# ska-sa/katsdpsigproc

Measured on AMD Instinct MI355X. Metric: visibility samples/s (baselines x channels) through full RFI flagger, higher is better.
Workload: dtype f32 amplitude / f64 deviations

## Files before the change

### katsdpsigproc_amd/csrc/fused_common.h

```cpp
#pragma once
#include <stdlib.h>

#include "bitplane.h"
#include "median_merge.h"
#include "median_window.h"

#ifndef FUSED_MAD_BITS
#define FUSED_MAD_BITS 1
#endif
#ifndef FUSED_STRIP
#define FUSED_STRIP 4
#endif
#define FUSED_THREADS (64 * FUSED_STRIP)
#define FUSED_MAD_NORMAL 1.4826

#ifdef KSP_DIAG_REALTIME
#define FUSED_DIAG_CLOCK() __builtin_amdgcn_s_memrealtime()
#else
#define FUSED_DIAG_CLOCK() __builtin_amdgcn_s_memtime()
#endif
#ifdef KSP_DIAG
#define FUSED_DIAG_STOP(p) ((p).debug_stop)
#define FUSED_DIAG_TRACE(p) ((p).trace)
#else
#define FUSED_DIAG_STOP(p) 0
#define FUSED_DIAG_TRACE(p) ((unsigned long long *)nullptr)
#endif

struct FusedParams {
    const void *vis;
    const uint8_t *in_flags;
    uint8_t *flags;
    float *deviations;
    float *noise;
    int channels, baselines;
    int vis_stride, in_flags_stride, flags_stride, dev_stride;
    int is_amplitude, flags_mode, threshold_kind, n_windows, flag_value;
    int n_strips;
    int n_static, n_dyn, dyn_blocks;
    unsigned *work;
    int first_round;
#ifdef KSP_DIAG
    int debug_stop;
    unsigned long long *trace;
#endif
    double n_sigma;
    double scales[KSP_MAX_WINDOWS];
};

template <int R>
struct FusedLayout {
    static constexpr int RUN = R + 4;
    static constexpr int ROW = 64 * RUN + 8;
    static constexpr int LDS_FLOATS = FUSED_STRIP * ROW;
    static constexpr int LIST_DOUBLES = 256;
    static constexpr size_t LDS_BYTES =
        sizeof(float) * LDS_FLOATS + sizeof(double) * LIST_DOUBLES * FUSED_STRIP;
    __device__ static __forceinline__ int index(int c) { return (c / R) * RUN + (c % R); }
};

#ifndef FUSED_XCD_GROUP
#define FUSED_XCD_GROUP 8
#endif
__device__ __forceinline__ int strip_of(int id, int n_strips)
{
    constexpr int G = FUSED_XCD_GROUP;
    const int full = (n_strips / (8 * G)) * (8 * G);
    if (id >= full) return id;
    const int xcd = id & 7, i = id >> 3;
    return ((i / G) * 8 + xcd) * G + (i % G);
}

__device__ __forceinline__ float amp_with_flags(const FusedParams &p, float re, float im,
                                                int row, int bl)
{
    float a = ksp_abs_c64(re, im);
    if (p.flags_mode == KSP_FLAGS_CHANNEL) {
        if (p.in_flags[row]) a = __builtin_nanf("");
    } else if (p.flags_mode == KSP_FLAGS_FULL) {
        if (p.in_flags[(size_t)row * p.in_flags_stride + bl]) a = __builtin_nanf("");
    }
    return a;
}

template <int R>
__device__ __forceinline__ void load_strip(const FusedParams &p, float *lds, int b0, int tid)
{
    using LY = FusedLayout<R>;
    constexpr int LB = 4;
    constexpr int LPR = FUSED_STRIP / 2;
    constexpr int RSTEP = FUSED_THREADS / LPR;
    const int C = p.channels;
    const int q = tid % LPR;
    const int r0 = tid / LPR;
    const int bl = b0 + 2 * q;
    const bool ok0 = bl < p.baselines, ok1 = bl + 1 < p.baselines;
    const bool plain = !p.is_amplitude && ok1;
    auto request = [&](float4 (&raw)[LB], unsigned (&fl)[LB], int rbase) {
#pragma unroll
        for (int u = 0; u < LB; u++) {
            const int row = rbase + u * RSTEP;
            raw[u] = make_float4(0.f, 0.f, 0.f, 0.f);
            fl[u] = 0;
            if (plain && row < C) {
                raw[u] = *(const float4 *)((const float2 *)p.vis + (size_t)row * p.vis_stride + bl);
                if (p.flags_mode == KSP_FLAGS_CHANNEL) {
                    fl[u] = p.in_flags[row];
                } else if (p.flags_mode == KSP_FLAGS_FULL) {
                    fl[u] = *(const unsigned short *)(p.in_flags + (size_t)row * p.in_flags_stride + bl);
                }
            }
        }
    };
    auto finish = [&](const float4 (&raw)[LB], const unsigned (&fl)[LB], int rbase) {
#pragma unroll
        for (int u = 0; u < LB; u++) {
            const int row = rbase + u * RSTEP;
            if (row >= C) break;
            float a0 = __builtin_nanf(""), a1 = __builtin_nanf("");
            unsigned fl8;
            if (plain) {
                a0 = ksp_abs_c64(raw[u].x, raw[u].y);
                a1 = ksp_abs_c64(raw[u].z, raw[u].w);
                if (p.flags_mode == KSP_FLAGS_CHANNEL) fl8 = fl[u] ? 0x101u : 0u; else fl8 = fl[u];
                if (fl8 & 0xffu) a0 = __builtin_nanf("");
                if (fl8 >> 8) a1 = __builtin_nanf("");
            } else if (p.is_amplitude) {
                const float *src = (const float *)p.vis + (size_t)row * p.vis_stride + bl;
                if (ok0) a0 = src[0];
                if (ok1) a1 = src[1];
                if (p.flags_mode == KSP_FLAGS_CHANNEL) {
                    if (p.in_flags[row]) a0 = a1 = __builtin_nanf("");
                } else if (p.flags_mode == KSP_FLAGS_FULL) {
                    const uint8_t *f = p.in_flags + (size_t)row * p.in_flags_stride + bl;
                    if (ok0 && f[0]) a0 = __builtin_nanf("");
                    if (ok1 && f[1]) a1 = __builtin_nanf("");
                }
            } else if (ok0) {
                const float2 v = ((const float2 *)p.vis)[(size_t)row * p.vis_stride + bl];
                a0 = amp_with_flags(p, v.x, v.y, row, bl);
            }
            const int idx = LY::index(row);
            lds[(2 * q) * LY::ROW + idx] = a0;
            lds[(2 * q + 1) * LY::ROW + idx] = a1;
        }
    };
    constexpr int BATCH = RSTEP * LB;
    float4 bufa[LB], bufb[LB];
    unsigned fla[LB], flb[LB];
    request(bufa, fla, r0);
    for (int rbase = r0; rbase < C; rbase += 2 * BATCH) {
        if (rbase + BATCH < C) request(bufb, flb, rbase + BATCH);
        finish(bufa, fla, rbase);
        if (rbase + BATCH < C) {
            if (rbase + 2 * BATCH < C) request(bufa, fla, rbase + 2 * BATCH);
            finish(bufb, flb, rbase + BATCH);
        }
    }
    for (int row = C + r0; row < 64 * R; row += RSTEP) {
        const int idx = LY::index(row);
        lds[(2 * q) * LY::ROW + idx] = __builtin_nanf("");
        lds[(2 * q + 1) * LY::ROW + idx] = __builtin_nanf("");
    }
}

#ifndef FUSED_LOAD_LB
#define FUSED_LOAD_LB 4
#endif
#ifndef FUSED_LOAD_NB
#define FUSED_LOAD_NB 3
#endif
template <int R, int MODE>
__device__ __forceinline__ bool load_strip_fast(const FusedParams &p, float *lds, int b0, int tid)
{
    using LY = FusedLayout<R>;
    constexpr int LB = FUSED_LOAD_LB;
    constexpr int LPR = FUSED_STRIP / 2;
    constexpr int RSTEP = FUSED_THREADS / LPR;
    constexpr int BATCH = RSTEP * LB;
    const int C = p.channels;
    const int q = tid % LPR;
    const int r0 = tid / LPR;
    const int bl = b0 + 2 * q;
    const float2 *vis = (const float2 *)p.vis + bl;
    const size_t stride = (size_t)p.vis_stride;
    unsigned umax = 0, flag_or = 0;
    auto request = [&](float4 (&raw)[LB], unsigned (&fl)[LB], int rbase) {
#pragma unroll
        for (int u = 0; u < LB; u++) {
            const int row = min(rbase + r0 + u * RSTEP, C - 1);
            raw[u] = *(const float4 *)(vis + (size_t)row * stride);
            fl[u] = 0;
            if (MODE == KSP_FLAGS_CHANNEL)
                fl[u] = p.in_flags[row];
            else if (MODE == KSP_FLAGS_FULL)
                fl[u] = *(const unsigned short *)(p.in_flags + (size_t)row * p.in_flags_stride + bl);
        }
    };
    auto finish = [&](const float4 (&raw)[LB], const unsigned (&fl)[LB], int rbase) {
        float amp[LB][2];
        if (FUSED_DIAG_STOP(p) == 11) {
#pragma unroll
            for (int u = 0; u < LB; u++) {
                amp[u][0] = raw[u].x;
                amp[u][1] = raw[u].z;
            }
        } else {
            ksp_abs_c64_batch<LB, MODE == KSP_FLAGS_NONE>(raw, amp, umax);
        }
#pragma unroll
        for (int u = 0; u < LB; u++) {
            const int row = rbase + r0 + u * RSTEP;
            float a0 = amp[u][0], a1 = amp[u][1];
            if (MODE == KSP_FLAGS_CHANNEL) {
                if (fl[u]) a0 = a1 = __builtin_nanf("");
            } else if (MODE == KSP_FLAGS_FULL) {
                if (fl[u] & 0xffu) a0 = __builtin_nanf("");
                if (fl[u] >> 8) a1 = __builtin_nanf("");
            }
            if (MODE != KSP_FLAGS_NONE) flag_or |= fl[u];
            if (row < C) {
                const int idx = LY::index(row);
                lds[(2 * q) * LY::ROW + idx] = a0;
                lds[(2 * q + 1) * LY::ROW + idx] = a1;
            }
        }
    };
    constexpr int NB = FUSED_LOAD_NB;
    float4 buf[NB][LB];
    unsigned fl[NB][LB];
#pragma unroll
    for (int k = 0; k < NB - 1; k++)
        if (k * BATCH < C) request(buf[k], fl[k], k * BATCH);
    for (int rb = 0; rb < C; rb += NB * BATCH) {
#pragma unroll
        for (int k = 0; k < NB; k++) {
            const int cur = rb + k * BATCH;
            if (cur < C) {
                const int ahead = cur + (NB - 1) * BATCH;
                if (ahead < C) request(buf[(k + NB - 1) % NB], fl[(k + NB - 1) % NB], ahead);
                finish(buf[k], fl[k], cur);
            }
        }
    }
    for (int row = C + r0; row < 64 * R; row += RSTEP) {
        const int idx = LY::index(row);
        lds[(2 * q) * LY::ROW + idx] = __builtin_nanf("");
        lds[(2 * q + 1) * LY::ROW + idx] = __builtin_nanf("");
    }
    return umax >= 0x7f800000u || flag_or != 0;
}

template <int R, int WIDTH, class Src>
__device__ __forceinline__ void median_phase_src(Src &&amp_rel, float (&dev)[R], float &dmax,
                                                 int *tiny = nullptr)
{
    constexpr int H = WIDTH / 2;
    dmax = -__builtin_inff();
    SortedWindow<WIDTH> win;
    win.reset();
    float ring[WIDTH];
#pragma unroll
    for (int j = -2 * H; j < R; j++) {
        const int k = 2 * H + j;
        const float a = amp_rel(H + j);
        if (k < WIDTH) {
            win.step_pad_out(a, __builtin_fabsf(a) < win.pinf);
        } else {
            float out = ring[k % WIDTH];
            asm("" : "+v"(out));
            win.step(out, __builtin_fabsf(out) < win.pinf, a, __builtin_fabsf(a) < win.pinf);
        }
        ring[k % WIDTH] = a;
        if (j >= 0) {
            float xc = ring[(k + WIDTH - H) % WIDTH];
            asm("" : "+v"(xc));
            float d = win.deviation(xc);
            d = (d == d) ? d : 0.0f;
            dmax = __builtin_amdgcn_fmed3f(dmax, d, win.pinf);
            dev[j] = d;
        }
    }
    if (tiny != nullptr) *tiny += win.tiny;
}

template <int R, int WIDTH>
__device__ __forceinline__ void median_phase(const float *myrow, int lane, float (&dev)[R],
                                             float &dmax, int *tiny = nullptr)
{
    using LY = FusedLayout<R>;
    constexpr int H = WIDTH / 2;
    const float *run = myrow + lane * LY::RUN;
    const float nan = __builtin_nanf("");
    auto amp_rel = [&](int i) -> float {
        if (i >= 0 && i < R) return run[i];
        if constexpr (H <= R) {
            if (i < 0) return lane > 0 ? run[i - (LY::RUN - R)] : nan;
            return lane < 63 ? run[i + (LY::RUN - R)] : nan;
        } else {
            const int c = lane * R + i;
            return (c >= 0 && c < 64 * R) ? myrow[LY::index(c)] : nan;
        }
    };
    median_phase_src<R, WIDTH>(amp_rel, dev, dmax, tiny);
}

template <int WIDTH, class Fetch>
__device__ __forceinline__ double exact_dev(int c, Fetch &&fetch)
{
    constexpr int H = WIDTH / 2;
    float pinf = __builtin_inff(), ninf = -__builtin_inff();
    asm volatile("" : "+v"(pinf), "+v"(ninf));
    float a[WIDTH];
#pragma unroll
    for (int k = 0; k < WIDTH; k++) a[k] = fetch(c - H + k);
    float v[WIDTH];
    int n = 0;
#pragma unroll
    for (int k = 0; k < WIDTH; k++) {
        const bool ok = __builtin_fabsf(a[k]) < pinf;
        n += ok;
        const float x = ok ? a[k] : pinf;
        float out[WIDTH];
        if (k == 0) {
            out[0] = x;
        } else {
            out[0] = __builtin_amdgcn_fmed3f(v[0], x, ninf);
#pragma unroll
            for (int i = 1; i < k; i++) out[i] = __builtin_amdgcn_fmed3f(v[i - 1], x, v[i]);
            out[k] = __builtin_amdgcn_fmed3f(v[k - 1], x, pinf);
        }
#pragma unroll
        for (int i = 0; i <= k; i++) v[i] = out[i];
    }
    const float centre = a[H];
    float lo = v[0], hi = v[0];
#pragma unroll
    for (int i = 0; i < WIDTH; i++) {
        lo = (i == ((n - 1) >> 1)) ? v[i] : lo;
        hi = (i == (n >> 1)) ? v[i] : hi;
    }
    if (!(centre == centre) || n == 0) return 0.0;
    const double med = (n & 1) ? (double)hi : ((double)lo + (double)hi) * 0.5;
    return (double)centre - med;
}

typedef unsigned short u16x2 __attribute__((ext_vector_type(2)));

template <int BITS>
__device__ __forceinline__ int wave_sum_small(int c)
{
    int total = 0;
#pragma unroll
    for (int b = 0; b < BITS; b++) total += __popcll(__ballot((c >> b) & 1)) << b;
    return total;
}

__device__ __forceinline__ int wave_max_int(int v)
{
#pragma unroll
    for (int off = 32; off > 0; off >>= 1) v = max(v, __shfl_xor(v, off, 64));
    return v;
}

template <int NP>
__device__ __forceinline__ int count_less16(const unsigned (&kp)[NP], unsigned T)
{
    const unsigned tc = ((T - 1) | 0x8000u) * 0x10001u;
    unsigned acc0 = 0, acc1 = 0;
#pragma unroll
    for (int i = 0; i < NP; i++) {
        const unsigned f = ((tc - kp[i]) >> 15) & 0x10001u;
        if (i & 1)
            acc1 += f;
        else
            acc0 += f;
    }
    const unsigned acc = acc0 + acc1;
    return wave_sum_small<7>((int)((acc & 0xffffu) + (acc >> 16)));
}

template <int WIDTH, class Fetch>
__device__ __forceinline__ int gather_exact(unsigned long long cand, int c0, double *list,
                                            int base, int cap, Fetch &&fetch)
{
    while (__any(cand != 0)) {
        const bool has = cand != 0;
        const int j = has ? __ffsll((long long)cand) - 1 : 0;
        cand &= cand - 1;
        const double x = fabs(exact_dev<WIDTH>(c0 + j, fetch));
        const unsigned long long m = __ballot(has);
        const int pos = base + __builtin_amdgcn_mbcnt_hi((unsigned)(m >> 32),
                                                         __builtin_amdgcn_mbcnt_lo((unsigned)m, 0));
        if (has && pos < cap) list[pos] = x;
        base += __popcll(m);
    }
    __builtin_amdgcn_fence(__ATOMIC_RELEASE, "wavefront");
    __builtin_amdgcn_wave_barrier();
    return base;
}

__device__ __forceinline__ void rank_in_list(const double *list, int n, int r, int lane,
                                             double &xk, double &prev, bool &have_prev)
{
    xk = 0.0;
    prev = 0.0;
    have_prev = false;
    if (n <= 64) {
        const bool live = lane < n;
        const double x = live ? list[lane] : 0.0;
        const int xlo = __double2loint(x), xhi = __double2hiint(x);
        int cnt = 0;
        for (int jj = 0; jj < n; jj++) {
            const double y = __hiloint2double(__builtin_amdgcn_readlane(xhi, jj),
                                              __builtin_amdgcn_readlane(xlo, jj));
            cnt += (y < x) || (y == x && jj < lane);
        }
        const unsigned long long hit = __ballot(live && cnt == r);
        const unsigned long long hitp = __ballot(live && cnt == r - 1);
        xk = __shfl(x, __ffsll((long long)hit) - 1, 64);
        if (hitp) {
            prev = __shfl(x, __ffsll((long long)hitp) - 1, 64);
            have_prev = true;
        }
        return;
    }
    for (int ci = lane; ci < ((n + 63) & ~63); ci += 64) {
        const bool live = ci < n;
        const double x = live ? list[ci] : 0.0;
        int cnt = 0;
        for (int jj = 0; jj < n; jj++) {
            const double y = list[jj];
            cnt += (y < x) || (y == x && jj < ci);
        }
        const unsigned long long hit = __ballot(live && cnt == r);
        const unsigned long long hitp = __ballot(live && cnt == r - 1);
        if (hit) xk = __shfl(x, __ffsll((long long)hit) - 1, 64);
        if (hitp) {
            prev = __shfl(x, __ffsll((long long)hitp) - 1, 64);
            have_prev = true;
        }
    }
}

__device__ __forceinline__ int ksp_bcast(int v, int src_lane)
{
    return __builtin_amdgcn_readlane(v, src_lane);
}
__device__ __forceinline__ float ksp_bcast(float v, int src_lane)
{
    return __builtin_bit_cast(float, __builtin_amdgcn_readlane(__builtin_bit_cast(int, v), src_lane));
}
__device__ __forceinline__ double ksp_bcast(double v, int src_lane)
{
    return __hiloint2double(__builtin_amdgcn_readlane(__double2hiint(v), src_lane),
                            __builtin_amdgcn_readlane(__double2loint(v), src_lane));
}

__device__ __forceinline__ void rank_lanes64(double x, int n, int r, int lane, double &xk,
                                             double &prev, bool &have_prev)
{
    const bool live = lane < n;
    const double xs = live ? x : __builtin_nan("");
    int cnt = 0;
#pragma unroll
    for (int blk = 0; blk < 64; blk += 8) {
        if (blk >= n) break;
#pragma unroll
        for (int u = 0; u < 8; u++) {
            const int jj = blk + u;
            const double y = ksp_bcast(xs, jj);
            cnt += (y < xs) || (y == xs && jj < lane);
        }
    }
    xk = ksp_bcast(x, __ffsll((long long)ksp_ballot(live && cnt == r)) - 1);
    have_prev = r >= 1;
    prev = have_prev ? ksp_bcast(x, __ffsll((long long)ksp_ballot(live && cnt == r - 1)) - 1) : 0.0;
}

__device__ __forceinline__ float ksp_select64(const float (&dev)[64], int j)
{
    auto pick = [](unsigned long long mask, float a, float b) -> float {
        float r;
        asm("v_cndmask_b32 %0, %1, %2, %3" : "=v"(r) : "v"(a), "v"(b), "s"(mask));
        return r;
    };
    const unsigned long long m0 = ksp_ballot(j & 1), m1 = ksp_ballot(j & 2), m2 = ksp_ballot(j & 4),
                             m3 = ksp_ballot(j & 8), m4 = ksp_ballot(j & 16), m5 = ksp_ballot(j & 32);
    float t32[32], t16[16], t8[8], t4[4];
#pragma unroll
    for (int i = 0; i < 32; i++) t32[i] = pick(m0, dev[2 * i], dev[2 * i + 1]);
#pragma unroll
    for (int i = 0; i < 16; i++) t16[i] = pick(m1, t32[2 * i], t32[2 * i + 1]);
#pragma unroll
    for (int i = 0; i < 8; i++) t8[i] = pick(m2, t16[2 * i], t16[2 * i + 1]);
#pragma unroll
    for (int i = 0; i < 4; i++) t4[i] = pick(m3, t8[2 * i], t8[2 * i + 1]);
    return pick(m5, pick(m4, t4[0], t4[1]), pick(m4, t4[2], t4[3]));
}
template <int R>
__device__ __forceinline__ float ksp_select_dev(const float (&dev)[R], int j)
{
    if constexpr (R == 64)
        return ksp_select64(dev, j);
    else
        return 0.0f;
}

__device__ __forceinline__ void rank_list_u32(const unsigned *vals, unsigned x, int n, int r,
                                              int lane, unsigned &xk, unsigned &prev,
                                              bool &have_prev)
{
    const bool live = lane < n;
    int lt = 0, le = 0;
#pragma unroll
    for (int blk = 0; blk < 64; blk += 8) {
        if (blk >= n) break;
        const uint4 a = *(const uint4 *)(vals + blk), b = *(const uint4 *)(vals + blk + 4);
        const unsigned y[8] = {a.x, a.y, a.z, a.w, b.x, b.y, b.z, b.w};
#pragma unroll
        for (int u = 0; u < 8; u++) {
            lt += y[u] < x;
            le += y[u] <= x;
        }
    }
    xk = (unsigned)__builtin_amdgcn_readlane(
        (int)x, __ffsll((long long)ksp_ballot(live && lt <= r && r < le)) - 1);
    have_prev = r >= 1;
    prev = have_prev ? (unsigned)__builtin_amdgcn_readlane(
                           (int)x, __ffsll((long long)ksp_ballot(live && lt <= r - 1 && r - 1 < le)) - 1)
                     : 0u;
}

template <int R, int WIDTH, int LIST_CAP, bool HAVE_EXACT = false, class Fetch>
__device__ __forceinline__ double mad_noise(const float (&dev)[R], int lane, double *list,
                                            Fetch &&fetch, int debug_stop = 0,
                                            unsigned long long *trace = nullptr,
                                            unsigned long long exact = 0, int *top_hint = nullptr,
                                            int tiny = 0)
{
    static_assert(!HAVE_EXACT || R == 64, "exactness masks are 64 bits, one per sample of a lane");
    constexpr int NP = R / 2;
    const int c0 = lane * R;
    auto dv = [&](int j) -> float {
        float x = dev[j];
        asm("" : "+v"(x));
        return x;
    };
    unsigned kp[NP];
#pragma unroll
    for (int i = 0; i < NP; i++) {
        const unsigned a = __float_as_uint(dev[2 * i]) + 0xffffu;
        const unsigned b = __float_as_uint(dev[2 * i + 1]) + 0xffffu;
        kp[i] = __builtin_amdgcn_perm(b, a, 0x07060302u) & 0x7fff7fffu;
    }
    int zeros;
    if constexpr (R != 64) zeros = count_less16<NP>(kp, 1);
    auto stamp = [&](int i) {
        if (trace != nullptr && lane == 0) trace[i] = FUSED_DIAG_CLOCK();
    };
    stamp(8);
    if (debug_stop == 31) return (double)(kp[0] + kp[NP - 1]);
    const int total = 64 * R;
    unsigned K = 0;
    int below_bin = 0, in_bin;
    int rank2 = 0, rank = 0;
    int zeros_keys = 0;
    unsigned eq0 = 0, eq1 = 0;
    if constexpr (R == 64) {
        unsigned np[32];
#pragma unroll
        for (int i = 0; i < 32; i++) np[i] = kp[i] ^ 0x7fff7fffu;
        transpose_bits32(np);
        stamp(9);
        {
            unsigned z0 = np[0], z1 = np[16];
#pragma unroll
            for (int b = 1; b < 15; b++) {
                z0 &= np[b];
                z1 &= np[16 + b];
            }
            zeros = ksp_wave_sum_dpp(__popc(z0) + __popc(z1));
        }
        zeros_keys = zeros;
        if (ksp_any(tiny != 0)) zeros -= ksp_wave_sum_dpp(tiny);
        if (zeros == total) return __builtin_nan("");
        rank2 = total + zeros;
        rank = rank2 / 2;
        if (rank < zeros_keys) return 0x1p-150 * FUSED_MAD_NORMAL;
        eq0 = eq1 = 0xffffffffu;
        auto step2 = [&](int hi, int lo) {
            const unsigned a0 = eq0 & np[hi], a1 = eq1 & np[16 + hi];
            const unsigned z00_0 = a0 & np[lo], z00_1 = a1 & np[16 + lo];
            const unsigned z01_0 = a0 ^ z00_0, z01_1 = a1 ^ z00_1;
            const unsigned b0 = eq0 ^ a0, b1 = eq1 ^ a1;
            const unsigned z10_0 = b0 & np[lo], z10_1 = b1 & np[16 + lo];
            const unsigned z11_0 = b0 ^ z10_0, z11_1 = b1 ^ z10_1;
            int s01 = (__popc(z00_0) + __popc(z00_1)) | ((__popc(z01_0) + __popc(z01_1)) << 16);
            int c10 = __popc(z10_0) + __popc(z10_1);
            ksp_wave_sum2_dpp(s01, c10);
            const int n1 = below_bin + (s01 & 0xffff), n2 = n1 + (s01 >> 16), n3 = n2 + c10;
            const bool g1 = n1 <= rank, g2 = n2 <= rank, g3 = n3 <= rank;
            K |= (unsigned)((int)g1 + (int)g2 + (int)g3) << lo;
            below_bin = g3 ? n3 : g2 ? n2 : g1 ? n1 : below_bin;
            eq0 = g3 ? z11_0 : g2 ? z10_0 : g1 ? z01_0 : z00_0;
            eq1 = g3 ? z11_1 : g2 ? z10_1 : g1 ? z01_1 : z00_1;
        };
        auto step1 = [&](int bit) {
            const unsigned z0 = eq0 & np[bit], z1 = eq1 & np[16 + bit];
            const int c = below_bin + ksp_wave_sum_dpp(__popc(z0) + __popc(z1));
            const bool take = c <= rank;
            K |= take ? (1u << bit) : 0u;
            below_bin = take ? c : below_bin;
            eq0 = take ? (eq0 ^ z0) : z0;
            eq1 = take ? (eq1 ^ z1) : z1;
        };
#if FUSED_MAD_BITS == 1
        bool hinted = false;
        if (top_hint != nullptr && *top_hint >= 0) {
            const unsigned h = (unsigned)*top_hint;
            unsigned e0 = 0xffffffffu, e1 = 0xffffffffu;
            int lb = 0;
#pragma unroll
            for (int bit = 14; bit >= 7; bit--) {
                const unsigned z0 = e0 & np[bit], z1 = e1 & np[16 + bit];
                if ((h >> (bit - 7)) & 1) {
                    lb += __popc(z0) + __popc(z1);
                    e0 ^= z0;
                    e1 ^= z1;
                } else {
                    e0 = z0;
                    e1 = z1;
                }
            }
            int cnt = __popc(e0) + __popc(e1);
            ksp_wave_sum2_dpp(lb, cnt);
            if (lb <= rank && rank < lb + cnt) {
                hinted = true;
                K = h << 7;
                below_bin = lb;
                eq0 = e0;
                eq1 = e1;
            }
        }
        if (hinted) {
#pragma unroll
            for (int bit = 6; bit >= 0; bit--) step1(bit);
        } else {
#pragma unroll
            for (int bit = 14; bit >= 0; bit--) step1(bit);
        }
        if (top_hint != nullptr) *top_hint = (int)(K >> 7);
#else
#pragma unroll
        for (int bit = 14; bit >= 2; bit -= 2) step2(bit, bit - 1);
        step1(0);
#endif
        in_bin = ksp_wave_sum_dpp(__popc(eq0) + __popc(eq1));
    } else {
        zeros_keys = zeros;
        if (ksp_any(tiny != 0)) zeros -= ksp_wave_sum(tiny);
        if (zeros == total) return __builtin_nan("");
        rank2 = total + zeros;
        rank = rank2 / 2;
        if (rank < zeros_keys) return 0x1p-150 * FUSED_MAD_NORMAL;
        for (int bit = 14; bit >= 0; bit--) {
            const unsigned test = K | (1u << bit);
            const int c = count_less16<NP>(kp, test);
            if (c <= rank) {
                K = test;
                below_bin = c;
            }
        }
        in_bin = count_less16<NP>(kp, K + 1) - below_bin;
    }
    const bool even = !(rank2 & 1);
    stamp(10);
    if (debug_stop == 32) return (double)(K + below_bin);
    auto key_of = [&](int j) -> unsigned {
        return min((__float_as_uint(dv(j)) & 0x7fffffffu) + 0xffffu, 0x7fffffffu) >> 16;
    };
    auto bin_mask = [&](unsigned key) -> unsigned long long {
        unsigned long long m = 0;
#pragma unroll
        for (int j = 0; j < R; j++)
            if (key_of(j) == key) m |= 1ull << j;
        return m;
    };
    int r = rank - below_bin;
    unsigned long long cand = 0;
    const bool narrowed = in_bin > LIST_CAP;
    if (narrowed) {
        const unsigned first = ((K - 1) << 16) + 1u;
        unsigned offs = 0;
        int below = below_bin;
        for (int bit = 15; bit >= 0; bit--) {
            const unsigned test = first + (offs | (1u << bit));
            int c = 0;
#pragma unroll
            for (int j = 0; j < R; j++) c += (__float_as_uint(dv(j)) & 0x7fffffffu) < test;
            c = ksp_wave_sum(c);
            if (c <= rank) {
                offs |= 1u << bit;
                below = c;
            }
        }
        const unsigned cur = first + offs;
        cand = 0;
#pragma unroll
        for (int j = 0; j < R; j++)
            if ((__float_as_uint(dv(j)) & 0x7fffffffu) == cur) cand |= 1ull << j;
        in_bin = ksp_wave_sum(__popcll(cand));
        r = rank - below;
        below_bin = below;
        if (in_bin > LIST_CAP) {
            auto each = [&](auto &&f) {
                unsigned long long todo = cand;
                while (__any(todo != 0)) {
                    const bool has = todo != 0;
                    const int j = has ? __ffsll((long long)todo) - 1 : 0;
                    todo &= todo - 1;
                    const double x = fabs(exact_dev<WIDTH>(c0 + j, fetch));
                    if (has) f(x);
                }
            };
            double lo = __builtin_inf(), hi = 0.0;
            each([&](double x) {
                lo = fmin(lo, x);
                hi = fmax(hi, x);
            });
            lo = ksp_wave_min(lo);
            hi = ksp_wave_max(hi);
            double xk = lo, prev = lo;
            if (lo != hi) {
                const unsigned long long base = (unsigned long long)__double_as_longlong(lo);
                const unsigned long long span = (unsigned long long)__double_as_longlong(hi) - base;
                unsigned long long offs = 0;
                int below_k = 0;
                for (int bit = 63 - __clzll((long long)span); bit >= 0; bit--) {
                    const unsigned long long test = base + (offs | (1ull << bit));
                    int c = 0;
                    each([&](double x) {
                        c += (unsigned long long)__double_as_longlong(x) < test;
                    });
                    c = ksp_wave_sum(c);
                    if (c <= r) {
                        offs |= 1ull << bit;
                        below_k = c;
                    }
                }
                xk = __longlong_as_double((long long)(base + offs));
                prev = xk;
                if (even && r >= 1 && below_k == r) {
                    double m = 0.0;
                    each([&](double x) { m = (x < xk) ? fmax(m, x) : m; });
                    prev = ksp_wave_max(m);
                }
            }
            if (even && r == 0) {
                float b32 = 0.0f;
#pragma unroll
                for (int j = 0; j < R; j++) {
                    const float a = fabsf(dv(j));
                    b32 = (__float_as_uint(a) < cur) ? fmaxf(b32, a) : b32;
                }
                b32 = ksp_wave_max(b32);
                unsigned long long bm = 0;
#pragma unroll
                for (int j = 0; j < R; j++)
                    if (fabsf(dv(j)) == b32) bm |= 1ull << j;
                const int n2 = gather_exact<WIDTH>(bm, c0, list, 0, LIST_CAP, fetch);
                double below_max = 0.0;
                for (int i = lane; i < min(n2, LIST_CAP); i += 64) below_max = fmax(below_max, list[i]);
                below_max = ksp_wave_max(below_max);
                __builtin_amdgcn_wave_barrier();
                if (n2 > LIST_CAP) {
                    unsigned long long todo = bm;
                    double m = 0.0;
                    while (__any(todo != 0)) {
                        const bool has = todo != 0;
                        const int j = has ? __ffsll((long long)todo) - 1 : 0;
                        todo &= todo - 1;
                        const double x = fabs(exact_dev<WIDTH>(c0 + j, fetch));
                        m = has ? fmax(m, x) : m;
                    }
                    below_max = ksp_wave_max(m);
                }
                prev = below_max;
            }
            if (even) xk = (xk + prev) / 2.0;
            return xk * FUSED_MAD_NORMAL;
        }
    }
    double xk, prev;
    bool have_prev;
    if (!narrowed && in_bin <= 64) {
        int *lc = (int *)list;
        int n = 0;
        auto place = [&](bool hit, int channel) {
            const unsigned long long m = ksp_ballot(hit);
            const int pos = n + __builtin_amdgcn_mbcnt_hi((unsigned)(m >> 32),
                                                         __builtin_amdgcn_mbcnt_lo((unsigned)m, 0));
            if (hit) lc[pos] = channel;
            n += __popcll(m);
        };
        double x;
        bool ranked = false;
        unsigned *lv = (unsigned *)lc + 128;
        static_assert(LIST_CAP * 2 >= 128 + 64 + 8, "candidate values behind the channel numbers");
        if constexpr (R == 64 && HAVE_EXACT) {
            const int mine = __popc(eq0) + __popc(eq1);
            const int incl = ksp_wave_scan_dpp(mine);
            n = __builtin_amdgcn_readlane(incl, 63);
            int pos = incl - mine;
            unsigned h0 = eq0, h1 = eq1;
            while (ksp_any((h0 | h1) != 0)) {
                const bool has = (h0 | h1) != 0;
                int j = 0;
                if (h0) {
                    j = 2 * (__ffs((int)h0) - 1);
                    h0 &= h0 - 1;
                } else if (h1) {
                    j = 2 * (__ffs((int)h1) - 1) + 1;
                    h1 &= h1 - 1;
                }
                const float v = ksp_select_dev<R>(dev, j);
                if (has) {
                    lc[pos] = (c0 + j) | (((exact >> j) & 1) ? (int)0x80000000 : 0);
                    lv[pos] = __float_as_uint(v) & 0x7fffffffu;
                    pos++;
                }
            }
            if (lane < 8) lv[n + lane] = 0xffffffffu;
            __builtin_amdgcn_fence(__ATOMIC_RELEASE, "wavefront");
            __builtin_amdgcn_wave_barrier();
            const int slot = lane < n ? lane : 0;
            const int e0 = lc[slot];
            const unsigned a32 = lv[slot];
            x = (double)__uint_as_float(a32);
            const bool inexact = lane < n && e0 >= 0;
            stamp(11);
            if (debug_stop == 33) return x;
            if (ksp_any(inexact)) {
                const double xe = fabs(exact_dev<WIDTH>(e0 & 0x7fffffff, fetch));
                x = inexact ? xe : x;
            } else {
                unsigned k32, p32;
                rank_list_u32(lv, a32, n, r, lane, k32, p32, have_prev);
                xk = (double)__uint_as_float(k32);
                prev = (double)__uint_as_float(p32);
                ranked = true;
            }
        } else {
            if constexpr (R == 64) {
                const int mine = __popc(eq0) + __popc(eq1);
                const int incl = ksp_wave_scan_dpp(mine);
                n = __builtin_amdgcn_readlane(incl, 63);
                int pos = incl - mine;
                unsigned h0 = eq0, h1 = eq1;
                while (h0 | h1) {
                    if (h0) {
                        lc[pos++] = c0 + 2 * (__ffs((int)h0) - 1);
                        h0 &= h0 - 1;
                    } else {
                        lc[pos++] = c0 + 2 * (__ffs((int)h1) - 1) + 1;
                        h1 &= h1 - 1;
                    }
                }
            } else {
#pragma unroll
                for (int j = 0; j < R; j++) place(key_of(j) == K, c0 + j);
            }
            __builtin_amdgcn_fence(__ATOMIC_RELEASE, "wavefront");
            __builtin_amdgcn_wave_barrier();
            const int c = lc[lane < n ? lane : 0];
            stamp(11);
            if (debug_stop == 33) return (double)c;
            x = fabs(exact_dev<WIDTH>(c, fetch));
        }
        stamp(12);
        if (!ranked) rank_lanes64(x, n, r, lane, xk, prev, have_prev);
        stamp(13);
        __builtin_amdgcn_wave_barrier();
    } else {
        gather_exact<WIDTH>(narrowed ? cand : bin_mask(K), c0, list, 0, LIST_CAP, fetch);
        rank_in_list(list, in_bin, r, lane, xk, prev, have_prev);
        __builtin_amdgcn_wave_barrier();
    }
    if (even && !have_prev) {
        int k2 = -1;
#pragma unroll
        for (int j = 0; j < R; j++) {
            const int kj = (int)key_of(j);
            k2 = (kj < (int)K) ? max(k2, kj) : k2;
        }
        k2 = wave_max_int(k2);
        const bool below_is_tiny = k2 <= 0;
        unsigned long long bm = bin_mask((unsigned)(below_is_tiny ? 0 : k2));
        float b32 = 0.0f;
#pragma unroll
        for (int j = 0; j < R; j++)
            if ((bm >> j) & 1) b32 = fmaxf(b32, fabsf(dv(j)));
        b32 = ksp_wave_max(b32);
        unsigned long long top = 0;
#pragma unroll
        for (int j = 0; j < R; j++)
            if (((bm >> j) & 1) && fabsf(dv(j)) == b32) top |= 1ull << j;
        bool recompute = true;
        if (below_is_tiny) {
            prev = 0x1p-150;
            recompute = false;
        }
        if constexpr (HAVE_EXACT) {
            if (recompute && !ksp_any((top & ~exact) != 0)) {
                prev = (double)b32;
                recompute = false;
            }
        }
        if (recompute) {
            const int n2 = gather_exact<WIDTH>(top, c0, list, 0, LIST_CAP, fetch);
            double below_max = 0.0;
            for (int i = lane; i < min(n2, LIST_CAP); i += 64) below_max = fmax(below_max, list[i]);
            prev = ksp_wave_max(below_max);
            __builtin_amdgcn_wave_barrier();
            if (n2 > LIST_CAP) {
                double m = 0.0;
                while (__any(top != 0)) {
                    const bool has = top != 0;
                    const int j = has ? __ffsll((long long)top) - 1 : 0;
                    top &= top - 1;
                    const double x = fabs(exact_dev<WIDTH>(c0 + j, fetch));
                    m = has ? fmax(m, x) : m;
                }
                prev = ksp_wave_max(m);
            }
        }
    }
    stamp(14);
    if (even) xk = (xk + prev) / 2.0;
    return xk * FUSED_MAD_NORMAL;
}

template <int WIDTH, class Fetch>
__device__ __noinline__ double exact_dev_call(int c, Fetch fetch)
{
    return exact_dev<WIDTH>(c, fetch);
}

template <int WIDTH, class Fetch>
__device__ __forceinline__ unsigned long long threshold_wide(const FusedParams &p,
                                                             const float (&dev)[64],
                                                             unsigned long long fl,
                                                             unsigned long long ge, double t1,
                                                             bool positive, int lane, int C,
                                                             Fetch &&fetch)
{
    const int c0 = lane * 64;
    float nmax = 0.0f;
#pragma unroll
    for (int j = 0; j < 64; j++) nmax = fmaxf(nmax, -dev[j]);
    nmax = ksp_wave_max(nmax);
    float U[64];
    unsigned Nb[16];
#pragma unroll
    for (int j = 0; j < 64; j++) U[j] = dev[j];
#pragma unroll
    for (int q = 0; q < 16; q++) Nb[q] = 0;
    int lvl = -1;
    float umax = 0.0f;
    bool counted = false;
    auto level = [&](auto s_) {
        constexpr int s = decltype(s_)::value;
        ksp_static_for<s>([&](auto r_) {
            constexpr int r = decltype(r_)::value;
            const float e = __shfl_down(U[r], 1, 64);
#pragma unroll
            for (int j = r; j + s < 64; j += s) U[j] += U[j + s];
            U[r + 64 - s] += e;
        });
        if (counted) {
            if constexpr (s >= 4) {
                constexpr int sq = s / 4;
                ksp_static_for<sq>([&](auto r_) {
                    constexpr int r = decltype(r_)::value;
                    const unsigned e = (unsigned)__shfl_down((int)Nb[r], 1, 64);
#pragma unroll
                    for (int q = r; q + sq < 16; q += sq) Nb[q] += Nb[q + sq];
                    Nb[r + 16 - sq] += e;
                });
            } else {
                const unsigned e = (unsigned)__shfl_down((int)Nb[0], 1, 64);
#pragma unroll
                for (int q = 0; q < 16; q++)
                    Nb[q] += __builtin_amdgcn_alignbyte(q + 1 < 16 ? Nb[(q + 1) % 16] : e, Nb[q], s);
            }
        }
    };
#pragma unroll 1
    for (int k = 0; k < p.n_windows; k++) {
        if (positive && !ksp_any((ge & ~fl) != 0)) break;
        const int w = 1 << k;
        const double scale = k == 0 ? p.scales[0] : k == 1 ? p.scales[1] : k == 2 ? p.scales[2]
                           : k == 3 ? p.scales[3] : k == 4 ? p.scales[4] : k == 5 ? p.scales[5]
                           : k == 6 ? p.scales[6] : p.scales[7];
        const float thrf = (float)(t1 * scale);
        const float limf = __fmul_rn(thrf, (float)w);
        const double limit = (double)limf;
        if (positive && lvl >= 0 && umax < thrf) continue;
        if (lvl < 0) {
            counted = ksp_any(fl != 0);
            {
                const unsigned f_lo = (unsigned)fl, f_hi = (unsigned)(fl >> 32);
#pragma unroll
                for (int j = 0; j < 64; j++)
                    U[j] = (((j < 32 ? f_lo : f_hi) >> (j & 31)) & 1u) ? 0.0f : dev[j];
            }
            float m = U[0];
#pragma unroll
            for (int j = 1; j < 64; j++) m = fmaxf(m, U[j]);
            umax = ksp_wave_max(m);
            if (counted) {
#pragma unroll
                for (int q = 0; q < 16; q++)
                    Nb[q] = ((((unsigned)(fl >> (4 * q))) & 0xfu) * 0x00204081u) & 0x01010101u;
            }
            lvl = 0;
            if (positive && umax < thrf) continue;
        }
        while (lvl < k) {
            switch (lvl) {
            case 0: level(std::integral_constant<int, 1>{}); break;
            case 1: level(std::integral_constant<int, 2>{}); break;
            case 2: level(std::integral_constant<int, 4>{}); break;
            case 3: level(std::integral_constant<int, 8>{}); break;
            case 4: level(std::integral_constant<int, 16>{}); break;
            case 5: level(std::integral_constant<int, 32>{}); break;
            default: level(std::integral_constant<int, 64>{}); break;
            }
            lvl++;
        }
        const int nvalid = C - w + 1 - c0;
        const unsigned long long valid = nvalid >= 64 ? ~0ull : nvalid <= 0 ? 0ull : ((1ull << nvalid) - 1);
        unsigned long long hits = 0, unsure = valid;
        if (positive) {
            unsigned h_lo = 0, h_hi = 0, m_lo = 0, m_hi = 0;
            const float c = (float)w * nmax * 0x1p-18f + (float)w * 0x1p-149f;
            if (counted) {
                const unsigned wq = (unsigned)w * 0x01010101u;
                auto one = [&](auto j_, unsigned &h, unsigned &m) {
                    constexpr int j = decltype(j_)::value;
                    const unsigned left = wq - Nb[j / 4];
                    const float rem = (float)((left >> (8 * (j % 4))) & 0xffu);
                    const float T = rem * thrf;
                    const float hi = __builtin_fmaf(T, 1.0f + 0x1p-18f, c);
                    float lo = __builtin_fmaf(T, 1.0f - 0x1p-18f, -c);
                    lo = (rem == 0.0f) ? __builtin_inff() : lo;
                    h = 2 * h + (U[j] > hi);
                    m = 2 * m + (U[j] > lo);
                };
                ksp_static_for<32>([&](auto i_) { one(std::integral_constant<int, 31 - decltype(i_)::value>{}, h_lo, m_lo); });
                ksp_static_for<32>([&](auto i_) { one(std::integral_constant<int, 63 - decltype(i_)::value>{}, h_hi, m_hi); });
            } else {
                const float hi = __builtin_fmaf(limf, 1.0f + 0x1p-18f, c);
                const float lo = __builtin_fmaf(limf, 1.0f - 0x1p-18f, -c);
#pragma unroll
                for (int j = 31; j >= 0; j--) {
                    h_lo = 2 * h_lo + (U[j] > hi);
                    m_lo = 2 * m_lo + (U[j] > lo);
                }
#pragma unroll
                for (int j = 63; j >= 32; j--) {
                    h_hi = 2 * h_hi + (U[j] > hi);
                    m_hi = 2 * m_hi + (U[j] > lo);
                }
            }
            hits = (((unsigned long long)h_hi << 32) | h_lo) & valid;
            unsure = (((unsigned long long)m_hi << 32) | m_lo) & valid & ~hits;
        }
        if (ksp_any(unsure != 0)) {
            const unsigned long long f1 = __shfl_down(fl, 1, 64), f2 = __shfl_down(fl, 2, 64);
            while (ksp_any(unsure != 0)) {
                const bool has = unsure != 0;
                const int j = has ? __ffsll((long long)unsure) - 1 : 0;
                unsure &= unsure - 1;
                double s = 0.0;
                for (int m = 0; m < w; m++) {
                    const int jj = j + m;
                    const unsigned long long fw = jj < 64 ? fl : jj < 128 ? f1 : f2;
                    const bool sub = (fw >> (jj & 63)) & 1;
                    const double x = exact_dev_call<WIDTH>(c0 + jj, fetch);
                    s += sub ? (double)thrf : x;
                }
                if (has && s > limit) hits |= 1ull << j;
            }
            lvl = -1;
        }
        if (!ksp_any(hits != 0)) continue;
        auto suffix_or = [](unsigned long long t) {
            t |= t >> 1; t |= t >> 2; t |= t >> 4; t |= t >> 8; t |= t >> 16; t |= t >> 32;
            return t;
        };
        unsigned long long add = hits;
        for (int s = 1; s < w && s < 64; s <<= 1) add |= add << s;
        unsigned long long h1 = __shfl_up(hits, 1, 64), h2 = __shfl_up(hits, 2, 64);
        if (lane < 1) h1 = 0;
        if (lane < 2) h2 = 0;
        if (w > 64) {
            add |= h1 ? ~0ull : 0ull;
            add |= suffix_or(h2 >> 1);
        } else if (w > 1) {
            add |= suffix_or(h1 >> (65 - w));
        }
        if (ksp_any((add & ~fl) != 0)) {
            fl |= add;
            lvl = -1;
        }
    }
    return fl;
}


template <int R, int WIDTH, int MAXK = 4, class Fetch>
__device__ __forceinline__ unsigned long long threshold_flags(const FusedParams &p,
                                                              const float (&dev)[R], float dmax,
                                                              double noise64, int lane, int C,
                                                              Fetch &&fetch)
{
    static_assert(R <= 64, "flag mask is 64 bits");
    const int c0 = lane * R;
    unsigned long long fl = 0;
    if (p.threshold_kind == KSP_THRESHOLD_SIMPLE) {
        const double thr = p.n_sigma * noise64;
        if (__any((double)dmax * (1.0 + 0x1p-23) > thr)) {
            unsigned long long unsure = 0;
#pragma unroll
            for (int j = 0; j < R; j++) {
                const double d = (double)dev[j];
                const double slack = fabs(d) * 0x1p-23 + 0x1p-149;
                if (d - slack > thr)
                    fl |= 1ull << j;
                else if (d + slack > thr)
                    unsure |= 1ull << j;
            }
            while (__any(unsure != 0)) {
                const bool has = unsure != 0;
                const int j = has ? __ffsll((long long)unsure) - 1 : 0;
                unsure &= unsure - 1;
                const double d = exact_dev<WIDTH>(c0 + j, fetch);
                if (has && d > thr) fl |= 1ull << j;
            }
        }
        return fl;
    }
    const double t1 = p.n_sigma * noise64;
    static_assert(MAXK == 4 || (MAXK == 8 && R == 64), "windows above 8: lanes of 64 channels");
    constexpr int MAXW = 4;
    float thr[MAXW];
    float thr_min = __builtin_inff();
    bool thr_nan = false;
#pragma unroll
    for (int k = 0; k < MAXK; k++) {
        const float t = (float)(t1 * p.scales[k < KSP_MAX_WINDOWS ? k : 0]);
        if (k < MAXW) thr[k < MAXW ? k : 0] = t;
        if (k < p.n_windows) {
            thr_min = fminf(thr_min, t);
            thr_nan |= (t != t);
        }
    }
    const double cand = (double)thr_min * (1.0 - 0x1p-20);
    const bool positive = thr_min > 0.0f;
    const bool any = !positive || ((double)dmax >= cand);
    if (thr_nan || !__any(any)) return 0;

    unsigned long long gt0, ge;
    {
        unsigned g_lo = 0, g_hi = 0, e_lo = 0, e_hi = 0;
        const float t0 = thr[0], tm = thr_min;
#pragma unroll
        for (int j = (R < 32 ? R : 32) - 1; j >= 0; j--)
            asm("v_cmp_ge_f32 vcc, %1, %2\n\tv_addc_co_u32 %0, vcc, %0, %0, vcc"
                : "+v"(e_lo) : "v"(dev[j]), "v"(tm) : "vcc");
#pragma unroll
        for (int j = R - 1; j >= 32; j--)
            asm("v_cmp_ge_f32 vcc, %1, %2\n\tv_addc_co_u32 %0, vcc, %0, %0, vcc"
                : "+v"(e_hi) : "v"(dev[j < R ? j : 0]), "v"(tm) : "vcc");
        if (ksp_any(dmax > t0)) {
#pragma unroll
            for (int j = (R < 32 ? R : 32) - 1; j >= 0; j--)
                asm("v_cmp_gt_f32 vcc, %1, %2\n\tv_addc_co_u32 %0, vcc, %0, %0, vcc"
                    : "+v"(g_lo) : "v"(dev[j]), "v"(t0) : "vcc");
#pragma unroll
            for (int j = R - 1; j >= 32; j--)
                asm("v_cmp_gt_f32 vcc, %1, %2\n\tv_addc_co_u32 %0, vcc, %0, %0, vcc"
                    : "+v"(g_hi) : "v"(dev[j < R ? j : 0]), "v"(t0) : "vcc");
        }
        gt0 = ((unsigned long long)g_hi << 32) | g_lo;
        ge = ((unsigned long long)e_hi << 32) | e_lo;
    }
    const unsigned long long inband =
        (c0 + R <= C) ? (R == 64 ? ~0ull : ((1ull << R) - 1))
                      : (c0 >= C ? 0ull : ((1ull << (C - c0)) - 1));
    if (positive && !__any(((ge & ~gt0) & inband) != 0)) return gt0 & inband;
    if constexpr (MAXK > 4) return threshold_wide<WIDTH>(p, dev, 0ull, ge, t1, positive, lane, C, fetch);

    float d[R];
#pragma unroll
    for (int j = 0; j < R; j++) d[j] = dev[j];
#pragma unroll
    for (int k = 0; k < MAXW; k++) {
        if (k >= p.n_windows) break;
        const int w = 1 << k;
        const float thrf = thr[k];
        const double limit = (double)__fmul_rn(thrf, (float)w);
        if (ksp_any(fl != 0)) {
#pragma unroll
            for (int j = 0; j < R; j++)
                if ((fl >> j) & 1) d[j] = thrf;
        }
        float ext[7];
#pragma unroll
        for (int m = 0; m < 7; m++) ext[m] = __shfl_down(d[m % R], 1 + m / R, 64);
        unsigned nfl = 0;
#pragma unroll
        for (int m = 0; m < 7; m++) {
            const unsigned long long f = __shfl_down(fl, 1 + m / R, 64);
            nfl |= (unsigned)((f >> (m % R)) & 1) << m;
        }
        unsigned long long need = ~0ull;
        if (positive && R == 64) {
            const unsigned long long hot = ge & ~fl;
            const unsigned long long hot_next = __shfl_down(hot, 1, 64);
            unsigned long long reach = hot;
#pragma unroll
            for (int m = 1; m < w; m++) reach |= (hot >> m) | (lane < 63 ? hot_next << (64 - m) : 0ull);
            need = ((unsigned long long)ksp_wave_or_dpp((unsigned)(reach >> 32)) << 32) |
                   ksp_wave_or_dpp((unsigned)reach);
        }
        unsigned long long hits = 0, unsure = 0;
#pragma unroll
        for (int j = 0; j < R; j++) {
            if (!((need >> j) & 1)) continue;
            double s = 0.0, mag = 0.0;
#pragma unroll
            for (int m = 0; m < w; m++) {
                {
                    const int jj = j + m;
                    const float v = (jj < R) ? d[jj % R] : ext[(jj >= R) ? (jj - R) % 7 : 0];
                    const bool sub = (jj < R) ? ((fl >> (jj % 64)) & 1) : ((nfl >> ((jj >= R) ? (jj - R) % 7 : 0)) & 1);
                    s += (double)v;
                    mag += sub ? 0.0 : fabs((double)v);
                }
            }
            const bool valid = (c0 + j + w <= C);
            const double slack = mag * 0x1p-23 + w * 0x1p-149;
            if (valid) {
                if (s - slack > limit)
                    hits |= 1ull << j;
                else if (s + slack > limit)
                    unsure |= 1ull << j;
            }
        }
        while (__any(unsure != 0)) {
            const bool has = unsure != 0;
            const int j = has ? __ffsll((long long)unsure) - 1 : 0;
            unsure &= unsure - 1;
            double s = 0.0;
            for (int m = 0; m < w; m++) {
                const int jj = j + m;
                const bool sub = (jj < R) ? ((fl >> jj) & 1) : ((nfl >> (jj - R)) & 1);
                const double x = exact_dev<WIDTH>(c0 + jj, fetch);
                s += sub ? (double)thrf : x;
            }
            if (has && s > limit) hits |= 1ull << j;
        }
        unsigned pin = 0;
        if (R >= 7) {
            const unsigned long long prev = __shfl_up(hits, 1, 64);
            if (lane > 0) pin = (unsigned)(prev >> (R >= 7 ? R - 7 : 0)) & 0x7fu;
        } else {
#pragma unroll
            for (int back = 1; back * R < 7 + R; back++) {
                const unsigned long long prev = __shfl_up(hits, back, 64);
                const int sh = 7 - back * R;
                if (lane >= back) pin |= (unsigned)(sh >= 0 ? (prev << sh) : (prev >> (-sh))) & 0x7fu;
            }
        }
        unsigned long long own = hits;
        if (w >= 2) { own |= own << 1; pin |= pin << 1; }
        if (w >= 4) { own |= own << 2; pin |= pin << 2; }
        if (w >= 8) { own |= own << 4; pin |= pin << 4; }
        const unsigned long long comb = own | (unsigned long long)(pin >> 7);
        fl |= comb & (R == 64 ? ~0ull : ((1ull << R) - 1));
    }
    return fl;
}

__device__ __forceinline__ void write_flags(const FusedParams &p, unsigned long long fl, int c0,
                                            int bl, int C)
{
    if (bl >= p.baselines) return;
    const uint8_t fv = (uint8_t)p.flag_value;
    while (fl) {
        const int j = __ffsll((long long)fl) - 1;
        fl &= fl - 1;
        const int c = c0 + j;
        if (c < C) p.flags[(size_t)c * p.flags_stride + bl] = fv;
    }
}
```

Before: 364.0 billion.

## Rank candidates before exact recompute and compute below-bin max with packed keys

The candidate-ranking path now always runs the u32 rank first, and only falls back to the exact f64 recompute when an inexact candidate actually lands on the selected rank or its predecessor. This avoids exact refetches in the common case. The even-median below-bin search is replaced with inline-asm packed-key max reductions and a carry-chain bitmask build, removing the separate key scan, bin mask and float max loops. It relies on a specific bit layout of the packed dev words and on a bias trick, which risks subtle correctness issues if that encoding differs.

Measured after the change: 389.8 billion (median of 6 runs). 7.1% higher.

```diff
diff --git a/katsdpsigproc_amd/csrc/fused_common.h b/katsdpsigproc_amd/csrc/fused_common.h
--- a/katsdpsigproc_amd/csrc/fused_common.h
+++ b/katsdpsigproc_amd/csrc/fused_common.h
@@ -841,12 +841,12 @@
             const bool inexact = lane < n && e0 >= 0;
             stamp(11);
             if (debug_stop == 33) return x;
-            if (ksp_any(inexact)) {
+            unsigned k32, p32;
+            rank_list_u32(lv, a32, n, r, lane, k32, p32, have_prev);
+            if (ksp_any(inexact && (a32 == k32 || (even && have_prev && a32 == p32)))) {
                 const double xe = fabs(exact_dev<WIDTH>(e0 & 0x7fffffff, fetch));
                 x = inexact ? xe : x;
             } else {
-                unsigned k32, p32;
-                rank_list_u32(lv, a32, n, r, lane, k32, p32, have_prev);
                 xk = (double)__uint_as_float(k32);
                 prev = (double)__uint_as_float(p32);
                 ranked = true;
@@ -888,24 +888,35 @@
         __builtin_amdgcn_wave_barrier();
     }
     if (even && !have_prev) {
-        int k2 = -1;
+        const unsigned bias = 0u - 2u * (((K - 1) << 16) + 1u);
+        unsigned wmax0 = bias, wmax1 = bias;
 #pragma unroll
         for (int j = 0; j < R; j++) {
-            const int kj = (int)key_of(j);
-            k2 = (kj < (int)K) ? max(k2, kj) : k2;
-        }
-        k2 = wave_max_int(k2);
-        const bool below_is_tiny = k2 <= 0;
-        unsigned long long bm = bin_mask((unsigned)(below_is_tiny ? 0 : k2));
-        float b32 = 0.0f;
-#pragma unroll
-        for (int j = 0; j < R; j++)
-            if ((bm >> j) & 1) b32 = fmaxf(b32, fabsf(dv(j)));
-        b32 = ksp_wave_max(b32);
+            unsigned w;
+            asm("v_lshl_add_u32 %0, %1, 1, %2" : "=v"(w) : "v"(dev[j]), "s"(bias));
+            if (j & 1)
+                wmax1 = max(wmax1, w);
+            else
+                wmax0 = max(wmax0, w);
+        }
+        const unsigned b2 = ksp_wave_max(max(wmax0, wmax1)) - bias;
+        const float b32 = __uint_as_float(b2 >> 1);
+        const bool below_is_tiny = b2 == 0;
         unsigned long long top = 0;
-#pragma unroll
-        for (int j = 0; j < R; j++)
-            if (((bm >> j) & 1) && fabsf(dv(j)) == b32) top |= 1ull << j;
+        if (!below_is_tiny) {
+            unsigned t_lo = 0, t_hi = 0, p2;
+#pragma unroll
+            for (int j = (R < 32 ? R : 32) - 1; j >= 0; j--)
+                asm("v_lshlrev_b32 %1, 1, %2\n\tv_cmp_eq_u32 vcc, %3, %1\n\t"
+                    "v_addc_co_u32 %0, vcc, %0, %0, vcc"
+                    : "+v"(t_lo), "=&v"(p2) : "v"(dev[j]), "s"(b2) : "vcc");
+#pragma unroll
+            for (int j = R - 1; j >= 32; j--)
+                asm("v_lshlrev_b32 %1, 1, %2\n\tv_cmp_eq_u32 vcc, %3, %1\n\t"
+                    "v_addc_co_u32 %0, vcc, %0, %0, vcc"
+                    : "+v"(t_hi), "=&v"(p2) : "v"(dev[j < R ? j : 0]), "s"(b2) : "vcc");
+            top = ((unsigned long long)t_hi << 32) | t_lo;
+        }
         bool recompute = true;
         if (below_is_tiny) {
             prev = 0x1p-150;
```
